# ross39/new_bloom_filter_repo

Hardware: AMD Instinct MI355X
Metric: Mpixels/s Bloom insert+query, 1080p residuals (higher is better)
Workload: dtype u64

## Files before the change

### include/rbf.h

```cpp
#ifndef RBF_H
#define RBF_H

#include <stddef.h>
#include <stdint.h>

#ifdef __cplusplus
extern "C" {
#endif

#define RBF_OK        0
#define RBF_EINVAL  (-22)
#define RBF_ENOMEM  (-12)
#define RBF_EIO      (-5)
#define RBF_ERANGE  (-34)

#define RBF_ABI_VERSION 4

typedef struct rbf_ctx rbf_ctx;

typedef struct {
    uint32_t m;
    uint32_t floor_k;
    uint64_t threshold;
} rbf_filter_params;

typedef struct {
    uint64_t h1;
    uint64_t h2;
    uint64_t act;
} rbf_seeds;

#define RBF_STAT_WITNESS_BITS 0
#define RBF_STAT_FILTER_ONES  1
#define RBF_STAT_RESERVED0    2
#define RBF_STAT_RESERVED1    3
#define RBF_STATS_PER_FRAME   4

int rbf_version(void);
const char *rbf_last_error(void);
int rbf_device_count(int *count);

int rbf_ctx_create(int device, void *hip_stream, rbf_ctx **out);
int rbf_ctx_destroy(rbf_ctx *ctx);
int rbf_ctx_sync(rbf_ctx *ctx);

int rbf_malloc(rbf_ctx *ctx, size_t bytes, void **out_dev);
int rbf_free(rbf_ctx *ctx, void *ptr_dev);
int rbf_memset(rbf_ctx *ctx, void *dst_dev, int value, size_t bytes);
int rbf_memcpy_h2d(rbf_ctx *ctx, void *dst_dev, const void *src, size_t bytes);
int rbf_memcpy_d2h(rbf_ctx *ctx, void *dst, const void *src_dev, size_t bytes);
int rbf_memcpy_d2d(rbf_ctx *ctx, void *dst_dev, const void *src_dev, size_t bytes);

#define RBF_K_MASK    0
#define RBF_K_INSERT  1
#define RBF_K_QUERY   2
#define RBF_K_STITCH  3
#define RBF_K_EXPAND  4
#define RBF_K_GATHER  5
#define RBF_K_SCATTER 6
#define RBF_K_INDEX   7
#define RBF_K_REDUCE  8
#define RBF_K_SCAN    9
#define RBF_K_NOISE   10
#define RBF_K_PACK    11
#define RBF_K_HASHTAB 12
#define RBF_K_HOLD    13
#define RBF_K_COUNT   14
int rbf_timing_enable(rbf_ctx *ctx, int on);
int rbf_ctx_force_generic(rbf_ctx *ctx, int on);
#define RBF_OPT_SEPARATE_FINISH 2
#define RBF_OPT_INSERT_SLICES 4
int rbf_ctx_option(rbf_ctx *ctx, int option, int64_t value);
int rbf_timing_reset(rbf_ctx *ctx);
int rbf_timing_read(rbf_ctx *ctx, int kernel_id, double *total_ms, uint64_t *launches);

int rbf_optimal_params(uint64_t n, uint64_t ones, double *k, uint64_t *l);
int rbf_activation_threshold(double k_star, uint32_t *floor_k, uint64_t *threshold);

int rbf_plan_batch(uint64_t n, const uint64_t *ones, uint32_t nframes, int guard_l_ge_n,
                   rbf_filter_params *params, double *k);

int rbf_residual_mask_batch(rbf_ctx *ctx, const void *frames_dev, uint64_t frame_stride_bytes,
                            uint32_t nframes, uint32_t width, uint32_t height,
                            uint64_t row_pitch_bytes, uint32_t pixel_stride_bytes,
                            uint32_t sample_bytes, int32_t thr_floor, const int32_t *thr_floors,
                            void *masks_dev, uint64_t mask_stride_bytes, uint64_t *ones_dev);

int rbf_residual_mask_batch_ex(rbf_ctx *ctx, const void *frames_dev, uint64_t frame_stride_bytes,
                               uint32_t nframes, uint32_t width, uint32_t height,
                               uint64_t row_pitch_bytes, uint32_t pixel_stride_bytes,
                               uint32_t sample_bytes, int32_t thr_floor, const int32_t *thr_floors,
                               void *masks_dev, uint64_t mask_stride_bytes, uint64_t *ones_dev, uint32_t mask_channels);

int rbf_temporal_hold_runs(rbf_ctx *ctx, void *frames_dev, uint64_t frame_stride_bytes, uint32_t nframes,
                           uint32_t width, uint32_t height, uint32_t channels, uint32_t sample_bytes,
                           uint32_t max_error, const uint8_t *run_starts);

int rbf_temporal_lookahead_runs(rbf_ctx *ctx, void *frames_dev, uint64_t frame_stride_bytes, uint32_t nframes,
                                uint32_t width, uint32_t height, uint32_t channels, uint32_t sample_bytes,
                                uint32_t max_error, const uint8_t *run_starts);

int rbf_temporal_hold_runs_map(rbf_ctx *ctx, void *frames_dev, uint64_t frame_stride_bytes, uint32_t nframes,
                               uint32_t width, uint32_t height, uint32_t channels, uint32_t sample_bytes,
                               const void *bounds_dev, const uint8_t *run_starts);
int rbf_temporal_lookahead_runs_map(rbf_ctx *ctx, void *frames_dev, uint64_t frame_stride_bytes, uint32_t nframes,
                                    uint32_t width, uint32_t height, uint32_t channels, uint32_t sample_bytes,
                                    const void *bounds_dev, const uint8_t *run_starts);

int rbf_bgr_to_gray_batch(rbf_ctx *ctx, const void *frames_dev, uint64_t frame_stride_bytes, uint32_t nframes,
                          uint32_t width, uint32_t height, uint64_t row_pitch_bytes, uint32_t pixel_stride_bytes,
                          uint32_t sample_bytes, void *gray_dev);

int rbf_extract_luma_batch(rbf_ctx *ctx, const void *frames_dev, uint64_t frame_stride_bytes, uint32_t nframes,
                           uint32_t width, uint32_t height, uint64_t row_pitch_bytes, uint32_t pixel_stride_bytes,
                           uint32_t sample_bytes, void *luma_dev);

int rbf_noise_moments_batch(rbf_ctx *ctx, const void *frames_dev, uint64_t frame_stride_bytes,
                            uint32_t nframes, uint32_t width, uint32_t height,
                            uint64_t row_pitch_bytes, uint32_t pixel_stride_bytes,
                            uint32_t sample_bytes, int64_t *moments_dev, float *noise_dev);


int rbf_bloom_encode_batch(rbf_ctx *ctx, const void *masks_dev, uint64_t mask_stride_bytes,
                           uint64_t n, uint32_t nframes, const rbf_filter_params *params,
                           const rbf_seeds *seeds,
                           void *filters_dev, uint64_t filter_stride_bytes,
                           void *witnesses_dev, uint64_t witness_stride_bytes,
                           uint64_t *stats_dev);

int rbf_encode_gop(rbf_ctx *ctx, const void *frames_dev, uint64_t frame_stride_bytes,
                   uint32_t nframes, uint32_t width, uint32_t height,
                   uint64_t row_pitch_bytes, uint32_t pixel_stride_bytes,
                   uint32_t sample_bytes, int32_t thr_floor, const int32_t *thr_floors,
                   const rbf_seeds *seeds,
                   void *masks_dev, uint64_t mask_stride_bytes, uint64_t *ones_dev,
                   void *filters_dev, uint64_t filter_stride_bytes,
                   void *witnesses_dev, uint64_t witness_stride_bytes, uint64_t *stats_dev,
                   rbf_filter_params *params_out, double *k_out);

int rbf_encode_gop_begin(rbf_ctx *ctx, const void *frames_dev, uint64_t frame_stride_bytes,
                         uint32_t nframes, uint32_t width, uint32_t height,
                         uint64_t row_pitch_bytes, uint32_t pixel_stride_bytes,
                         uint32_t sample_bytes, int32_t thr_floor, const int32_t *thr_floors,
                         const rbf_seeds *seeds,
                         void *masks_dev, uint64_t mask_stride_bytes, uint64_t *ones_dev,
                         void *filters_dev, uint64_t filter_stride_bytes,
                         void *witnesses_dev, uint64_t witness_stride_bytes, uint64_t *stats_dev);
int rbf_encode_gop_poll(rbf_ctx *ctx, int *ready);

#define RBF_PAIR_SKIPPED 0xFFFFFFFFu
uint64_t rbf_filter_stride_min(uint64_t n);
int rbf_encode_runs_begin(rbf_ctx *ctx, const void *frames_dev, uint64_t frame_stride_bytes,
                          uint32_t nframes, uint32_t width, uint32_t height,
                          uint64_t row_pitch_bytes, uint32_t pixel_stride_bytes,
// ... 118 lines not shown
```

### new_bloom_filter_repo_amd/_native.py

```python
import ctypes
import os
import weakref

import numpy as np

_HERE = os.path.dirname(os.path.abspath(__file__))
LIB_PATH = os.environ.get("RBF_LIB_PATH") or os.path.join(_HERE, "librbf_hip.so")

RBF_OK = 0
RBF_EINVAL = -22
RBF_ENOMEM = -12
RBF_EIO = -5
RBF_ERANGE = -34

K_MASK, K_INSERT, K_QUERY, K_STITCH, K_EXPAND, K_GATHER, K_SCATTER, K_INDEX, K_REDUCE, K_SCAN, K_NOISE, K_PACK, K_HASHTAB, K_HOLD = range(14)
KERNEL_NAMES = ["mask", "insert", "query", "stitch", "expand", "gather", "scatter", "index", "reduce", "scan", "noise", "pack", "hashtab", "hold"]
STATS_PER_FRAME = 4
PAIR_SKIPPED = 0xFFFFFFFF
OPT_SEPARATE_FINISH, OPT_INSERT_SLICES = 2, 4


class FilterParams(ctypes.Structure):
    _fields_ = [("m", ctypes.c_uint32), ("floor_k", ctypes.c_uint32), ("threshold", ctypes.c_uint64)]


ERROR_ROW = np.dtype([("sse", "<u8"), ("differing", "<u8"), ("over_bound", "<u8"), ("max_abs", "<u4"), ("reserved", "<u4")])
SWEEP_ROW = np.dtype([("sse", "<u8"), ("updates", "<u8"), ("max_abs", "<u4"), ("reserved", "<u4")])
SWEEP_MAX_CANDIDATES = 8
PAN_ROW = np.dtype([("dx", "<i4"), ("dy", "<i4"), ("sad_zero", "<u8"), ("sad_best", "<u8"), ("moving_zero", "<u8"), ("moving_best", "<u8")])
PAN_MAX_RANGE = 32


class Seeds(ctypes.Structure):
    _fields_ = [("h1", ctypes.c_uint64), ("h2", ctypes.c_uint64), ("act", ctypes.c_uint64)]


class RbfError(RuntimeError):
    def __init__(self, code, msg):
        super().__init__("librbf_hip error %d: %s" % (code, msg))
        self.code = code


_vp, _u64, _u32, _i32, _int = ctypes.c_void_p, ctypes.c_uint64, ctypes.c_uint32, ctypes.c_int32, ctypes.c_int
_i32p = ctypes.POINTER(ctypes.c_int32)
_PROTOS = {
    "rbf_version": (_int, []),
    "rbf_last_error": (ctypes.c_char_p, []),
    "rbf_device_count": (_int, [ctypes.POINTER(_int)]),
    "rbf_ctx_create": (_int, [_int, _vp, ctypes.POINTER(_vp)]),
    "rbf_ctx_destroy": (_int, [_vp]),
    "rbf_ctx_sync": (_int, [_vp]),
    "rbf_malloc": (_int, [_vp, ctypes.c_size_t, ctypes.POINTER(_vp)]),
    "rbf_free": (_int, [_vp, _vp]),
    "rbf_memset": (_int, [_vp, _vp, _int, ctypes.c_size_t]),
    "rbf_memcpy_h2d": (_int, [_vp, _vp, _vp, ctypes.c_size_t]),
    "rbf_memcpy_d2h": (_int, [_vp, _vp, _vp, ctypes.c_size_t]),
    "rbf_memcpy_d2d": (_int, [_vp, _vp, _vp, ctypes.c_size_t]),
    "rbf_timing_enable": (_int, [_vp, _int]),
    "rbf_timing_reset": (_int, [_vp]),
    "rbf_ctx_force_generic": (_int, [_vp, _int]),
    "rbf_ctx_option": (_int, [_vp, _int, ctypes.c_int64]),
    "rbf_timing_read": (_int, [_vp, _int, ctypes.POINTER(ctypes.c_double), ctypes.POINTER(_u64)]),
    "rbf_optimal_params": (_int, [_u64, _u64, ctypes.POINTER(ctypes.c_double), ctypes.POINTER(_u64)]),
    "rbf_activation_threshold": (_int, [ctypes.c_double, ctypes.POINTER(_u32), ctypes.POINTER(_u64)]),
    "rbf_plan_batch": (_int, [_u64, ctypes.POINTER(_u64), _u32, _int, ctypes.POINTER(FilterParams), ctypes.POINTER(ctypes.c_double)]),
    "rbf_encode_gop": (_int, [_vp, _vp, _u64, _u32, _u32, _u32, _u64, _u32, _u32, _i32, _i32p, ctypes.POINTER(Seeds),
                              _vp, _u64, _vp, _vp, _u64, _vp, _u64, _vp, ctypes.POINTER(FilterParams), ctypes.POINTER(ctypes.c_double)]),
    "rbf_encode_gop_begin": (_int, [_vp, _vp, _u64, _u32, _u32, _u32, _u64, _u32, _u32, _i32, _i32p, ctypes.POINTER(Seeds),
                                    _vp, _u64, _vp, _vp, _u64, _vp, _u64, _vp]),
    "rbf_encode_gop_poll": (_int, [_vp, ctypes.POINTER(_int)]),
    "rbf_filter_stride_min": (_u64, [_u64]),
    "rbf_encode_runs_begin": (_int, [_vp, _vp, _u64, _u32, _u32, _u32, _u64, _u32, _u32, _i32, _i32p, _vp, ctypes.POINTER(Seeds),
                                     _vp, _u64, _vp, _vp, _u64, _vp, _u64, _vp]),
    "rbf_encode_runs_begin_ex": (_int, [_vp, _vp, _u64, _u32, _u32, _u32, _u64, _u32, _u32, _i32, _i32p, _vp, ctypes.POINTER(Seeds),
                                        _vp, _u64, _vp, _vp, _u64, _vp, _u64, _vp, _u32]),
    "rbf_encode_runs": (_int, [_vp, _vp, _u64, _u32, _u32, _u32, _u64, _u32, _u32, _i32, _i32p, _vp, ctypes.POINTER(Seeds),
                               _vp, _u64, _vp, _vp, _u64, _vp, _u64, _vp, ctypes.POINTER(FilterParams), ctypes.POINTER(ctypes.c_double)]),
    "rbf_encode_gop_finish": (_int, [_vp, ctypes.POINTER(FilterParams), ctypes.POINTER(ctypes.c_double)]),
    "rbf_residual_mask_batch": (_int, [_vp, _vp, _u64, _u32, _u32, _u32, _u64, _u32, _u32, _i32, _i32p, _vp, _u64, _vp]),
    "rbf_residual_mask_batch_ex": (_int, [_vp, _vp, _u64, _u32, _u32, _u32, _u64, _u32, _u32, _i32, _i32p, _vp, _u64, _vp, _u32]),
    "rbf_temporal_hold_runs": (_int, [_vp, _vp, _u64, _u32, _u32, _u32, _u32, _u32, _u32, _vp]),
    "rbf_temporal_lookahead_runs": (_int, [_vp, _vp, _u64, _u32, _u32, _u32, _u32, _u32, _u32, _vp]),
    "rbf_temporal_hold_runs_map": (_int, [_vp, _vp, _u64, _u32, _u32, _u32, _u32, _u32, _vp, _vp]),
    "rbf_temporal_lookahead_runs_map": (_int, [_vp, _vp, _u64, _u32, _u32, _u32, _u32, _u32, _vp, _vp]),
    "rbf_record_max_bytes": (_u64, [_u32, _u64]),
    "rbf_pack_records": (_int, [_vp, _u32, _u64, ctypes.POINTER(FilterParams), ctypes.POINTER(ctypes.c_double),
                                _vp, _u64, _vp, _u64, _vp, _u64, _vp, _vp, _u64]),
    "rbf_gather_values_batch": (_int, [_vp, _vp, _u64, _u32, _u32, _u32, _u64, _u32, _u32, _u32, _vp, _u64, _vp, _u64, _vp, _vp]),
    "rbf_bgr_to_gray_batch": (_int, [_vp, _vp, _u64, _u32, _u32, _u32, _u64, _u32, _u32, _vp]),
    "rbf_extract_luma_batch": (_int, [_vp, _vp, _u64, _u32, _u32, _u32, _u64, _u32, _u32, _vp]),
    "rbf_noise_moments_batch": (_int, [_vp, _vp, _u64, _u32, _u32, _u32, _u64, _u32, _u32, _vp, _vp]),
    "rbf_bloom_encode_batch": (_int, [_vp, _vp, _u64, _u64, _u32, ctypes.POINTER(FilterParams), ctypes.POINTER(Seeds),
                                      _vp, _u64, _vp, _u64, _vp]),
    "rbf_bloom_decode_batch": (_int, [_vp, _vp, _u64, _vp, _u64, _u64, _u32, ctypes.POINTER(FilterParams),
                                      ctypes.POINTER(Seeds), _vp, _u64]),
    "rbf_filter_insert_indices": (_int, [_vp, _vp, ctypes.POINTER(FilterParams), ctypes.POINTER(Seeds), _vp, _u64]),
    "rbf_filter_query_indices": (_int, [_vp, _vp, ctypes.POINTER(FilterParams), ctypes.POINTER(Seeds), _vp, _u64, _vp]),
    "rbf_filter_insert_keys": (_int, [_vp, _vp, ctypes.POINTER(FilterParams), ctypes.POINTER(Seeds), _u32, _vp, _vp, _u64]),
    "rbf_filter_query_keys": (_int, [_vp, _vp, ctypes.POINTER(FilterParams), ctypes.POINTER(Seeds), _u32, _vp, _vp, _u64, _vp]),
    "rbf_gather_values": (_int, [_vp, _vp, _u32, _u32, _u64, _u32, _u32, _u32, _vp, _vp, _vp]),
    "rbf_scatter_values": (_int, [_vp, _vp, _u32, _u32, _u64, _u32, _u32, _u32, _vp, _vp]),
# ... 218 lines not shown
```

### new_bloom_filter_repo_amd/csrc/rbf_api.hip

```cpp
#include "rbf_host.h"
#include "rbf_kernels.h"
#include "rbf_kernels_noise.h"
#include "rbf_kernels_mask.h"
#include "rbf_kernels_hold.h"
#include "rbf_kernels_lookahead.h"
#include "rbf_kernels_barrett.h"
#include "rbf_kernels_insert_f64.h"
#include "rbf_kernels_reduce.h"
#include "rbf_kernels_query_f64.h"
#include "rbf_kernels_query_f64_tiled.h"
#include "rbf_kernels_witness.h"
#include "rbf_kernels_pack.h"
#include "rbf_kernels_digest.h"
#include "rbf_kernels_cut.h"
#include "rbf_kernels_error.h"
#include "rbf_kernels_sweep.h"
#include "rbf_kernels_pan.h"
#include "rbf_kernels_view.h"
#include "rbf_rice_host.h"
#include "rbf_kernels_keyquant.h"

#include <cmath>
#include <cstring>

// ... 341 lines not shown
            if (b.params[f].m) first += ones_host[f];
        }
        if (int r = launch_insert_positions(ctx, b, itab, sd, hashed_positions)) return r;
    }
    for (uint32_t f0 = 0; f0 < nframes;) {
        SliceTable grp{};
        uint32_t per_tile = 0, coded = 0, f = f0;
        for (; f < nframes && coded < pl.insert_group; ++f) {
            grp.n[f] = pl.slices.n[f];
            per_tile += grp.n[f];
            coded += grp.n[f] ? 1u : 0u;
        }
        f0 = f;
        if (!per_tile) continue;
        const dim3 grid(per_tile * pl.insert_tiles), block(IL_THREADS);
        LaunchTimer t(ctx, RBF_K_INSERT);
        if (two_phase)
            hipLaunchKernelGGL(k_insert_records, grid, block, pl.insert_lds_bytes, ctx->stream, (const uint2 *)ctx->ins_records.p,
                               (const uint32_t *)ctx->ins_counters.p, rtab, ctx->partials.p, part_stride, pl.insert_tile_words, grp, per_tile, pl.S);
        else if (use_tab)
            hipLaunchKernelGGL(tkern, grid, block, pl.insert_lds_bytes, ctx->stream, (const uint8_t *)b.masks, b.mask_stride, b.n, itab, hash_tab, sd,
                               ctx->partials.p, part_stride, pl.insert_tile_words, grp, per_tile, pl.S);
        else
            hipLaunchKernelGGL(ikern, grid, block, pl.insert_lds_bytes, ctx->stream, (const uint8_t *)b.masks, b.mask_stride, b.n, tab, sd,
                               ctx->partials.p, part_stride, pl.insert_tile_words, grp, per_tile, pl.S);
    }
    LaunchTimer t(ctx, RBF_K_REDUCE);
    const uint64_t words = b.filter_stride / 4;
    const uint32_t vec_ok = (words % 4 == 0 && ((uintptr_t)b.filters % 16) == 0) ? 1u : 0u;
    const uint32_t bx = std::max(1u, (uint32_t)((words + WG_THREADS * 4 - 1) / (WG_THREADS * 4)));
    hipLaunchKernelGGL(stream_once ? k_filter_reduce<true> : k_filter_reduce<false>, dim3(bx, nframes), dim3(WG_THREADS), 0, ctx->stream,
                       (const uint32_t *)ctx->partials.p, part_stride, pl.S, pl.slices, tab, (uint32_t *)b.filters, words, b.stats, vec_ok, image,
                       (uint64_t)pl.image_stride_words);
    return RBF_OK;
}

static int insert_generic(rbf_ctx *ctx, const Plan &pl, const BloomBatch &b, const FrameTable &tab, uint32_t *image)
{
    HIP_TRY(hipMemsetAsync(b.filters, 0, (size_t)b.nframes * b.filter_stride, ctx->stream));
    const uint64_t words = b.filter_stride / 4;
    const uint64_t bx = std::min<uint64_t>(((b.n + 31) / 32 + WG_THREADS - 1) / WG_THREADS, 65535);
    {
        LaunchTimer t(ctx, RBF_K_INSERT);
        hipLaunchKernelGGL(k_insert, dim3((uint32_t)bx, b.nframes), dim3(WG_THREADS), 0, ctx->stream, (const uint32_t *)b.masks, b.mask_stride / 4,
                           b.n, tab, to_dev(*b.seeds), (uint32_t *)b.filters, words);
    }
    LaunchTimer t(ctx, RBF_K_REDUCE);
    SliceTable ones;
    memset(ones.n, 1, sizeof ones.n);
    const uint32_t bx2 = std::max(1u, (uint32_t)((words + WG_THREADS * 4 - 1) / (WG_THREADS * 4)));
    hipLaunchKernelGGL(k_filter_reduce<false>, dim3(bx2, b.nframes), dim3(WG_THREADS), 0, ctx->stream, (const uint32_t *)b.filters, words, 1u, ones,
                       tab, (uint32_t *)b.filters, words, b.stats, 0u, image, (uint64_t)pl.image_stride_words);
    return RBF_OK;
}

static int encode_chunk_pass(rbf_ctx *ctx, const BloomBatch &b, bool outputs_zeroed, const uint64_t *ones_host, bool quiet_passthrough, bool compact)
{
    const uint32_t nframes = b.nframes;
    uint64_t nrecords = 0;
    uint32_t coded = 0;
    for (uint32_t f = 0; f < nframes; ++f) {
        if (!b.params[f].m) continue;
        ++coded;
        if (ones_host) nrecords += ones_host[f];
    }
    Plan pl = make_plan(ctx->knobs, ctx->cus, b.params, nframes, b.n, ones_host && nrecords < (1ull << 32));
    if (pl.insert_two_phase &&
        (ctx->ins_records.reserve((size_t)(nrecords ? nrecords : 1) * 8) || ctx->ins_counters.reserve((size_t)MAX_BATCH * 4))) {
        (void)hipGetLastError();
        pl = make_plan(ctx->knobs, ctx->cus, b.params, nframes, b.n, false);
    }
    FrameTable tab;
    if (int r = fill_table(b.params, nframes, &tab)) return r;
    const bool stream_once = (uint64_t)coded * b.n >= STREAM_MIN_PIXEL_FRAMES;
    if (int r = reserve_query_outputs(ctx, pl, nframes)) return r;
    if (int r = ctx->seg_off.reserve((size_t)nframes * pl.nseg * 8)) return r;
    const bool want_image = pl.reads_probe_image();
    if (want_image) if (int r = ctx->qimage.reserve((size_t)nframes * pl.image_stride_words * 4)) return r;
    uint32_t *image = want_image ? ctx->qimage.p : nullptr;
    if (!outputs_zeroed)
        HIP_TRY(hipMemsetAsync(b.stats, 0, (size_t)nframes * RBF_STATS_PER_FRAME * 8, ctx->stream));
    if (int r = pl.fast_insert ? insert_fast(ctx, pl, b, tab, ones_host, stream_once, image) : insert_generic(ctx, pl, b, tab, image)) return r;
    if (int r = launch_query(ctx, pl, b, tab, QueryFlags{want_image, pl.insert_tab, quiet_passthrough})) return r;
    if (compact) {
        uint32_t bx;
        if (int r = launch_chunk_offsets(ctx, pl, nframes, &bx, b.witnesses, b.witness_stride)) return r;
        LaunchTimer t(ctx, RBF_K_STITCH);
        hipLaunchKernelGGL(stream_once ? k_compact_witness<true> : k_compact_witness<false>, dim3(bx, nframes), dim3(WG_THREADS), 0, ctx->stream,
                           ctx->pass_words.p, ctx->seg_cnt.p, pl.nseg, pl.words_per_seg, (const uint64_t *)b.masks, b.mask_stride / 8, b.n,
                           (uint32_t *)b.witnesses, b.witness_stride / 4, b.stats, ctx->chunk_off.p);
    }
    HIP_TRY(hipGetLastError());
    return RBF_OK;
}

static int encode_chunk(rbf_ctx *ctx, const BloomBatch &b, bool outputs_zeroed, const uint64_t *ones_host)
{
    rbf_filter_params small[MAX_BATCH], big[MAX_BATCH];
    if (ctx->knobs.fp64_kernels() && !ctx->knobs.no_hash_table && split_by_family(b.params, b.nframes, small, big)) {
        const Plan ps = make_plan(ctx->knobs, ctx->cus, small, b.nframes, b.n, false);
        const Plan pb = make_plan(ctx->knobs, ctx->cus, big, b.nframes, b.n, ones_host != nullptr);
        if (pb.reads_probe_image() && pb.insert_tab && ps.nseg == pb.nseg && ps.words_per_seg == pb.words_per_seg) {
            if (int r = encode_chunk_pass(ctx, b.with(small), outputs_zeroed, nullptr, false, false)) return r;
            return encode_chunk_pass(ctx, b.with(big), true, ones_host, true, true);
        }
    }
    return encode_chunk_pass(ctx, b, outputs_zeroed, ones_host, false, true);
}

static int encode_batch_impl(rbf_ctx *ctx, const BloomBatch &b, bool outputs_zeroed, const uint64_t *ones_host = nullptr)
{
    if (int r = set_device(ctx)) return r;
    if (!b.masks || !b.params || !b.seeds || !b.filters || !b.witnesses || !b.stats) return fail(RBF_EINVAL, "null pointer");
    if (int r = check_frame_geometry(b.n, b.nframes, b.mask_stride)) return r;
    if (int r = check_filter_strides(b.params, b.nframes, b.filter_stride)) return r;
    if (int r = check_witness_stride(b.n, b.witness_stride)) return r;
    if (int r = check_base8(b.masks, "masks_dev")) return r;
    if (int r = check_base8(b.filters, "filters_dev")) return r;
    if (int r = check_base8(b.witnesses, "witnesses_dev")) return r;
    if (int r = check_base8(b.stats, "stats_dev")) return r;
    for (uint32_t f0 = 0; f0 < b.nframes; f0 += MAX_BATCH) {
        const uint32_t cnt = std::min(b.nframes - f0, (uint32_t)MAX_BATCH);
        if (int r = encode_chunk(ctx, b.rows(f0, cnt), outputs_zeroed, ones_host ? ones_host + f0 : nullptr)) return r;
    }
    return RBF_OK;
}

static int decode_chunk(rbf_ctx *ctx, const BloomBatch &b)
{
    const uint32_t nframes = b.nframes;
    const Plan pl = make_plan(ctx->knobs, ctx->cus, b.params, nframes, b.n);
    FrameTable tab;
    if (int r = fill_table(b.params, nframes, &tab)) return r;
    if (int r = reserve_query_outputs(ctx, pl, nframes)) return r;
    bool split = false;
    rbf_filter_params small[MAX_BATCH], big[MAX_BATCH];
    if (ctx->knobs.fp64_kernels() && split_by_family(b.params, nframes, small, big)) {
        const Plan ps = make_plan(ctx->knobs, ctx->cus, small, nframes, b.n), pb = make_plan(ctx->knobs, ctx->cus, big, nframes, b.n);
        if (pb.reads_probe_image() && ps.nseg == pl.nseg && pb.nseg == pl.nseg && ps.words_per_seg == pl.words_per_seg &&
            pb.words_per_seg == pl.words_per_seg) {
            FrameTable ts, tb;
            if (int r = fill_table(small, nframes, &ts)) return r;
            if (int r = fill_table(big, nframes, &tb)) return r;
            if (int r = launch_query(ctx, ps, b, ts, QueryFlags{})) return r;
            if (int r = launch_query(ctx, pb, b, tb, QueryFlags{false, false,  true})) return r;
            split = true;
        }
    }
    if (!split) if (int r = launch_query(ctx, pl, b, tab, QueryFlags{})) return r;
    uint32_t bx;
    if (int r = launch_chunk_offsets(ctx, pl, nframes, &bx)) return r;
    LaunchTimer t(ctx, RBF_K_EXPAND);
    hipLaunchKernelGGL(k_expand_mask, dim3(bx, nframes), dim3(WG_THREADS), 0, ctx->stream, ctx->pass_words.p, ctx->seg_cnt.p, pl.nseg,
                       pl.words_per_seg, (const uint32_t *)b.witnesses, b.witness_stride / 4, (uint64_t *)b.masks, b.mask_stride / 8, b.n,
                       ctx->chunk_off.p);
    HIP_TRY(hipGetLastError());
    return RBF_OK;
}

static LayoutRules frame_pass_rules(uint32_t samples)
{
    LayoutRules r;
    r.samples = samples; r.min_frames = 1; r.max_frames = 65535;
    return r;
}

template <class KernelOf>
// ... 116 lines not shown
    HIP_TRY(hipStreamSynchronize(ctx->stream));
    return RBF_OK;
}

int rbf_malloc(rbf_ctx *ctx, size_t bytes, void **out_dev)
{
    if (int r = set_device(ctx)) return r;
    if (!out_dev) return fail(RBF_EINVAL, "out_dev is null");
    *out_dev = nullptr;
    if (bytes == 0) bytes = 8;
    hipError_t e = hipMalloc(out_dev, bytes);
    if (e != hipSuccess) return fail(e == hipErrorOutOfMemory ? RBF_ENOMEM : RBF_EIO, "hipMalloc(%zu): %s", bytes, hipGetErrorString(e));
    return RBF_OK;
}

int rbf_free(rbf_ctx *ctx, void *ptr_dev)
{
    if (int r = set_device(ctx)) return r;
    if (!ptr_dev) return RBF_OK;
    HIP_TRY(hipStreamSynchronize(ctx->stream));
    HIP_TRY(hipFree(ptr_dev));
    return RBF_OK;
}

int rbf_memset(rbf_ctx *ctx, void *dst_dev, int value, size_t bytes)
{
    if (int r = set_device(ctx)) return r;
    if (bytes == 0) return RBF_OK;
    if (!dst_dev) return fail(RBF_EINVAL, "dst_dev is null");
    HIP_TRY(hipMemsetAsync(dst_dev, value, bytes, ctx->stream));
    return RBF_OK;
}

int rbf_memcpy_h2d(rbf_ctx *ctx, void *dst_dev, const void *src, size_t bytes)
{
    if (int r = set_device(ctx)) return r;
    if (bytes == 0) return RBF_OK;
    if (!dst_dev || !src) return fail(RBF_EINVAL, "null pointer");
    HIP_TRY(hipMemcpyAsync(dst_dev, src, bytes, hipMemcpyHostToDevice, ctx->stream));
    HIP_TRY(hipStreamSynchronize(ctx->stream));
    return RBF_OK;
}

int rbf_memcpy_d2h(rbf_ctx *ctx, void *dst, const void *src_dev, size_t bytes)
{
    if (int r = set_device(ctx)) return r;
    if (bytes == 0) return RBF_OK;
    if (!dst || !src_dev) return fail(RBF_EINVAL, "null pointer");
    HIP_TRY(hipMemcpyAsync(dst, src_dev, bytes, hipMemcpyDeviceToHost, ctx->stream));
    HIP_TRY(hipStreamSynchronize(ctx->stream));
    return RBF_OK;
}

int rbf_memcpy_d2d(rbf_ctx *ctx, void *dst_dev, const void *src_dev, size_t bytes)
{
    if (int r = set_device(ctx)) return r;
    if (bytes == 0) return RBF_OK;
    if (!dst_dev || !src_dev) return fail(RBF_EINVAL, "null pointer");
    HIP_TRY(hipMemcpyAsync(dst_dev, src_dev, bytes, hipMemcpyDeviceToDevice, ctx->stream));
    return RBF_OK;
}

int rbf_timing_enable(rbf_ctx *ctx, int on)
{
    if (int r = set_device(ctx)) return r;
    if (!on) { if (int r = drain_timing(ctx)) return r; }
    ctx->timing = on == 1 ? 0xFFFFFFFFu : (uint32_t)on;
    return RBF_OK;
}

int rbf_ctx_force_generic(rbf_ctx *ctx, int on)
{
    if (!ctx) return fail(RBF_EINVAL, "null context");
    ctx->knobs.set_flags(on);
    return RBF_OK;
}

int rbf_ctx_option(rbf_ctx *ctx, int option, int64_t value)
{
    if (!ctx) return fail(RBF_EINVAL, "null context");
    switch (option) {
    case RBF_OPT_SEPARATE_FINISH: ctx->knobs.no_fused_finish = value != 0; return RBF_OK;
    case RBF_OPT_INSERT_SLICES: ctx->knobs.insert_slices = value < 0 ? 0u : (uint32_t)value; return RBF_OK;
    default: return fail(RBF_EINVAL, "unknown option %d", option);
    }
}

int rbf_timing_reset(rbf_ctx *ctx)
{
    if (int r = set_device(ctx)) return r;
    if (int r = drain_timing(ctx)) return r;
    for (int k = 0; k < RBF_K_COUNT; ++k) { ctx->total_ms[k] = 0; ctx->launches[k] = 0; }
    return RBF_OK;
}

int rbf_timing_read(rbf_ctx *ctx, int kernel_id, double *total_ms, uint64_t *launches)
{
    if (int r = set_device(ctx)) return r;
    if (kernel_id < 0 || kernel_id >= RBF_K_COUNT) return fail(RBF_EINVAL, "kernel id %d", kernel_id);
    if (int r = drain_timing(ctx)) return r;
    if (total_ms) *total_ms = ctx->total_ms[kernel_id];
    if (launches) *launches = ctx->launches[kernel_id];
    return RBF_OK;
}

int rbf_optimal_params(uint64_t n, uint64_t ones, double *k_out, uint64_t *l_out)
{
    if (!k_out || !l_out) return fail(RBF_EINVAL, "null output");
    *k_out = 0.0; *l_out = 0;
    if (n == 0 || ones > n) return fail(RBF_EINVAL, "need 0 <= ones <= n, n > 0");
    const double p = (double)ones / (double)n;
    if (p <= 0.0001) return RBF_OK;
    if (p >= 0.32453) return RBF_OK;
    const double q = 1 - p;
    const double L = std::log(2.0);
    const double k = std::log2(q * std::pow(L, 2.0) / p);
    if (std::isnan(k) || k <= 0) return RBF_OK;
    const double gamma = 1 / L;
    const double lf = p * (double)n * k * gamma;
    const uint64_t l = (uint64_t)lf;
    *k_out = k > 0.1 ? k : 0.1;
    *l_out = l > 1 ? l : 1;
    return RBF_OK;
}

int rbf_activation_threshold(double k_star, uint32_t *floor_k, uint64_t *threshold)
{
    if (!floor_k || !threshold) return fail(RBF_EINVAL, "null output");
    if (!(k_star >= 0.0) || k_star > 64.0) return fail(RBF_ERANGE, "k* = %g outside [0, 64]", k_star);
    const double fl = std::floor(k_star);
    *floor_k = (uint32_t)fl;
    const double pa = k_star - fl;
    if (!(pa > 0.0)) { *threshold = 0; return RBF_OK; }
    int ex;
    const double fr = std::frexp(pa, &ex);
    const uint64_t A = (uint64_t)std::ldexp(fr, 53);
    const int s = ex - 53 - 2;
    const uint64_t N = (A == (1ull << 52)) ? 4 * A - 1 : 4 * A - 2;
    const int sh = -s;
    if (sh >= 128) { *threshold = 1; return RBF_OK; }
    const unsigned __int128 X = (unsigned __int128)N * (unsigned __int128)0xFFFFFFFFFFFFFFFFull;
    *threshold = (uint64_t)(X >> sh) + 1;
    return RBF_OK;
}

int rbf_plan_batch(uint64_t n, const uint64_t *ones, uint32_t nframes, int guard_l_ge_n,
                   rbf_filter_params *params, double *k_out)
{
    if (!ones || !params) return fail(RBF_EINVAL, "null pointer");
    for (uint32_t f = 0; f < nframes; ++f) {
        double k = 0.0; uint64_t l = 0;
        if (int r = rbf_optimal_params(n, ones[f], &k, &l)) return r;
        const bool skip = (l == 0) || (guard_l_ge_n && l >= n) || l > 0xFFFFFFFFull;
        params[f].m = 0; params[f].floor_k = 0; params[f].threshold = 0;
        if (!skip) {
            params[f].m = (uint32_t)l;
            if (int r = rbf_activation_threshold(k, &params[f].floor_k, &params[f].threshold)) return r;
        }
        if (k_out) k_out[f] = skip ? 0.0 : k;
    }
    return RBF_OK;
}

int rbf_residual_mask_batch(rbf_ctx *ctx, const void *frames_dev, uint64_t frame_stride_bytes,
                            uint32_t nframes, uint32_t width, uint32_t height,
                            uint64_t row_pitch_bytes, uint32_t pixel_stride_bytes,
// ... 1070 lines not shown
```

### new_bloom_filter_repo_amd/csrc/rbf_kernels_witness.h

```cpp
#pragma once
#include "rbf_kernels.h"

namespace rbf {

constexpr int CO_THREADS = 1024;
__global__ __launch_bounds__(CO_THREADS) void k_chunk_offsets(const uint32_t *__restrict__ seg_cnt, uint64_t nseg, uint32_t chunk_segs, uint32_t nchunks,
                                                              uint32_t *__restrict__ off, uint32_t *__restrict__ witnesses , uint64_t witness_stride_words32)
{
    __shared__ uint32_t wtot[CO_THREADS / WAVE];
    __shared__ uint32_t carry_s;
    const uint32_t f = blockIdx.x;
    const uint32_t lane = threadIdx.x & 63u, wave = threadIdx.x >> 6;
    const uint32_t *cnt = seg_cnt + (uint64_t)f * nseg;
    uint32_t *out = off + (uint64_t)f * nchunks;
    uint32_t *wit = witnesses ? witnesses + (uint64_t)f * witness_stride_words32 : nullptr;
    auto zero_word_at = [&](uint32_t bit) {
        const uint64_t d = (bit >> 5) & ~1u;
        if (d < witness_stride_words32) wit[d] = 0;
        if (d + 1 < witness_stride_words32) wit[d + 1] = 0;
    };
    const uint32_t per = (chunk_segs & 3u) == 0 ? 4u : (chunk_segs & 1u) == 0 ? 2u : 1u;
    if (threadIdx.x == 0) carry_s = 0;
    __syncthreads();
    for (uint64_t base = 0; base < nseg; base += (uint64_t)CO_THREADS * per) {
// ... 61 lines not shown
        off += __popc(p4);
    }
    return out;
}
__device__ __forceinline__ uint32_t pdep32_lut(const uint8_t *lut, uint32_t w, uint32_t p)
{
    uint32_t out = 0, off = 0;
#pragma unroll
    for (int j = 0; j < 8; ++j) {
        const uint32_t p4 = __builtin_amdgcn_ubfe(p, 4u * j, 4u), w4 = __builtin_amdgcn_ubfe(w, off, 4u);
        out |= (uint32_t)lut[(p4 << 4) | w4] << (4u * j);
        off += __popc(p4);
    }
    return out;
}

template <bool STREAM>
__global__ __launch_bounds__(WG_THREADS) void k_compact_witness(
    const uint64_t *__restrict__ pass_words, const uint32_t *__restrict__ seg_cnt, uint64_t nseg, uint32_t words_per_seg,
    const uint64_t *__restrict__ masks, uint64_t mask_stride_words64, uint64_t n,
    uint32_t *__restrict__ witnesses, uint64_t witness_stride_words32, uint64_t *__restrict__ stats,
    const uint32_t *__restrict__ chunk_off )
{
    __shared__ uint32_t buf[WG_THREADS * 2 + 2];
    __shared__ uint32_t wsum[WG_WAVES];
    __shared__ __attribute__((aligned(4))) uint8_t lut[256];
    const uint32_t f = blockIdx.y;
    const uint32_t lane = threadIdx.x & 63u, wave = __builtin_amdgcn_readfirstlane(threadIdx.x >> 6);
    const uint32_t nwords = (uint32_t)((n + 63) >> 6);
    const uint32_t total = (uint32_t)nseg * words_per_seg;
    const uint64_t *pwf = pass_words + (uint64_t)f * total;
    const uint32_t start32 = chunk_off[(uint64_t)f * gridDim.x + blockIdx.x];
    uint32_t *wit = witnesses + (uint64_t)f * witness_stride_words32;
    const uint32_t wbeg = blockIdx.x * WG_THREADS;
    const uint32_t w = wbeg + threadIdx.x;
    const bool have = w < total && w < nwords;
    const uint64_t *mkp = masks + (uint64_t)f * mask_stride_words64 + w;
    const uint64_t pw_raw = have ? (STREAM ? __builtin_nontemporal_load(pwf + w) : pwf[w]) : 0ull;
    const uint64_t mk_raw = have ? (STREAM ? __builtin_nontemporal_load(mkp) : *mkp) : 0ull;
    lut_to_lds(lut, LUT_PEXT4);
    buf[threadIdx.x] = 0;
    buf[threadIdx.x + WG_THREADS] = 0;
    if (threadIdx.x < 2) buf[threadIdx.x + 2 * WG_THREADS] = 0;
    const uint64_t pw = flip_bytes64(pw_raw);
    const uint32_t pw_lo = (uint32_t)pw, pw_hi = (uint32_t)(pw >> 32);
    const uint32_t c_lo = __popc(pw_lo), c = c_lo + __popc(pw_hi);
    const uint32_t incl = wave_inclusive_scan(c);
    if (lane == WAVE - 1) wsum[wave] = incl;
    __syncthreads();
    uint32_t before = 0, chunk_total = 0;
#pragma unroll
    for (int k = 0; k < WG_WAVES; ++k) {
        if ((uint32_t)k < wave) before += wsum[k];
        chunk_total += wsum[k];
    }
    const uint32_t obase = start32 & ~31u;
    const uint32_t o = start32 + before + incl - c;
    const uint64_t mk = flip_bytes64(mk_raw);
    const uint32_t o_lo = pext32_lut(lut, (uint32_t)mk, pw_lo), o_hi = pext32_lut(lut, (uint32_t)(mk >> 32), pw_hi);
    const uint64_t out = (uint64_t)o_lo | ((uint64_t)o_hi << c_lo);
    if (out) {
        const uint32_t rel = o - obase;
        const uint32_t sh = rel & 31u, word = rel >> 5;
        const uint32_t lo = (uint32_t)out, hi = (uint32_t)(out >> 32);
        const uint32_t d0 = lo << sh;
        const uint32_t d1 = sh ? ((lo >> (32u - sh)) | (hi << sh)) : hi;
        const uint32_t d2 = sh ? (hi >> (32u - sh)) : 0u;
        if (d0) atomicOr(&buf[word], d0);
        if (d1) atomicOr(&buf[word + 1], d1);
        if (d2) atomicOr(&buf[word + 2], d2);
    }
    __syncthreads();
    const uint32_t oend = start32 + chunk_total;
    const uint32_t ndw = ((oend - obase) + 31u) >> 5;
    for (uint32_t i = threadIdx.x; i < ndw; i += WG_THREADS) {
        const uint32_t v = buf[i];
        const bool shared = (i == 0 && (start32 & 31u)) || (i + 1 == ndw && (oend & 31u));
        if (shared) { if (v) atomicOr(&wit[(obase >> 5) + i], flip_bytes32(v)); }
        else wit[(obase >> 5) + i] = flip_bytes32(v);
    }
    if (threadIdx.x == 0 && wbeg + WG_THREADS >= total) stats[(uint64_t)f * 4 + 0] = oend;
}

__global__ __launch_bounds__(WG_THREADS) void k_expand_mask(
    const uint64_t *__restrict__ pass_words, const uint32_t *__restrict__ seg_cnt, uint64_t nseg, uint32_t words_per_seg,
    const uint32_t *__restrict__ witnesses, uint64_t witness_stride_words32,
    uint64_t *__restrict__ masks, uint64_t mask_stride_words64, uint64_t n, const uint32_t *__restrict__ chunk_off )
{
    __shared__ uint32_t wsum[WG_WAVES];
    __shared__ __attribute__((aligned(4))) uint8_t lut[256];
    const uint32_t f = blockIdx.y;
    const uint32_t lane = threadIdx.x & 63u, wave = __builtin_amdgcn_readfirstlane(threadIdx.x >> 6);
    const uint32_t nwords = (uint32_t)((n + 63) >> 6);
    const uint32_t total = (uint32_t)nseg * words_per_seg;
    const uint32_t start32 = chunk_off[(uint64_t)f * gridDim.x + blockIdx.x];
    const uint32_t *wit = witnesses + (uint64_t)f * witness_stride_words32;
    const uint32_t wbeg = blockIdx.x * WG_THREADS;
    const uint32_t w = wbeg + threadIdx.x;
    const bool have = w < total && w < nwords;
    const uint64_t pw_raw = have ? pass_words[(uint64_t)f * total + w] : 0ull;
    lut_to_lds(lut, LUT_PDEP4);
    const uint64_t p = flip_bytes64(pw_raw);
    const uint32_t p_lo = (uint32_t)p, p_hi = (uint32_t)(p >> 32);
    const uint32_t c_lo = __popc(p_lo), c = c_lo + __popc(p_hi);
    const uint32_t incl = wave_inclusive_scan(c);
    if (lane == WAVE - 1) wsum[wave] = incl;
    __syncthreads();
    uint32_t o = start32 + incl - c;
#pragma unroll
    for (int k = 0; k < WG_WAVES; ++k)
        if ((uint32_t)k < wave) o += wsum[k];
    if (w >= nwords) return;
    uint64_t out = 0;
    if (c) {
        const uint32_t d0 = o >> 5, dl = (o + c - 1u) >> 5, r = o & 31u;
        const uint64_t x0 = d0 < witness_stride_words32 ? flip_bytes32(wit[d0]) : 0u;
        const uint64_t x1 = (d0 + 1 <= dl && d0 + 1 < witness_stride_words32) ? flip_bytes32(wit[d0 + 1]) : 0u;
        const uint64_t x2 = (d0 + 2 <= dl && d0 + 2 < witness_stride_words32) ? flip_bytes32(wit[d0 + 2]) : 0u;
        uint64_t win = (x0 | (x1 << 32)) >> r;
        win |= r ? x2 << (64u - r) : 0ull;
        out = (uint64_t)pdep32_lut(lut, (uint32_t)win, p_lo) | ((uint64_t)pdep32_lut(lut, (uint32_t)(win >> c_lo), p_hi) << 32);
    }
    masks[(uint64_t)f * mask_stride_words64 + w] = flip_bytes64(out);
}

}
```

### new_bloom_filter_repo_amd/csrc/rbf_plan.h

```cpp
#pragma once
#include "../../include/rbf.h"
#include "rbf_geometry.h"

#include <algorithm>
#include <cstring>

using namespace rbf;

static int fail(int code, const char *fmt, ...);

struct Knobs {
    bool force_generic = false;
    bool single_buffer = false;
    bool force_generic_mask_bits = false;
    bool barrett_only = false;
    bool hash_rebuild = false;
    bool no_hash_table = false;
    bool no_two_phase = false;
    bool hash_positions = false;
    bool no_table_rewrite = false;
    bool no_fused_finish = false;
    uint32_t mask_chunks = 0;
    uint32_t tile_words = 0;
    uint32_t insert_slices = 0;
    void set_flags(int on)
    {
        force_generic = on & 1;
        single_buffer = on & 2;
        force_generic_mask_bits = on & 4;
        barrett_only = on & 8;
        hash_rebuild = on & 16;
        no_hash_table = on & 32;
        no_two_phase = on & 128;
        mask_chunks = (uint32_t)(on >> 8) & 0x1F;
        hash_positions = on & (1 << 14);
        no_table_rewrite = on & (1 << 15);
        tile_words = ((uint32_t)on >> 16) << 6;
    }
    bool fp64_kernels() const { return !force_generic && !barrett_only && !single_buffer; }
};

static inline FrameDev frame_dev(const rbf_filter_params &p)
{
    return FrameDev{p.m, p.floor_k, p.threshold, p.m >= 2 ? (uint64_t)((((unsigned __int128)1) << 64) / p.m) : 0};
}

static int fill_table(const rbf_filter_params *params, uint32_t count, FrameTable *tab)
{
    memset(tab, 0, sizeof *tab);
    for (uint32_t f = 0; f < count; ++f) {
        if (params[f].floor_k > 64) return fail(RBF_ERANGE, "frame %u: floor_k %u > 64", f, params[f].floor_k);
        tab->f[f] = frame_dev(params[f]);
    }
    return RBF_OK;
}

static FrameTable query_table(const FrameTable &tab, uint32_t nframes, U64Classes *cls, uint32_t *nactive, uint64_t (&empty)[2])
{
    FrameTable q;
    memset(&q, 0, sizeof q);
    if (cls) memset(cls, 0, sizeof *cls);
    empty[0] = empty[1] = 0;
    uint64_t sorted[MAX_BATCH];
    uint32_t coded = 0;
    for (uint32_t f = 0; f < nframes; ++f) {
        if (tab.f[f].m) sorted[coded++] = tab.f[f].T;
        else empty[f >> 6] |= 1ull << (f & 63);
    }
    std::sort(sorted, sorted + coded);
    uint32_t j = 0;
    for (int k = 0; k < (cls ? U64_CLASSES : 1); ++k)
        for (uint32_t f = 0; f < nframes; ++f) {
            if (!tab.f[f].m) continue;
            const uint32_t fk = tab.f[f].floor_k;
            if (cls && (fk >= 1u && fk <= 5u ? (int)fk - 1 : 5) != k) continue;
            const double ninv = -1.0 / (double)tab.f[f].m;
            const uint32_t below = (uint32_t)(std::lower_bound(sorted, sorted + coded, tab.f[f].T) - sorted);
            q.f[j].m = tab.f[f].m;
            memcpy(&q.f[j].M, &ninv, 8);
            q.f[j].floor_k = (fk & 0xFFu) | (below << 8) | (f << 16);
            q.f[j].T = sorted[j];
            if (cls) ++cls->n[k];
            ++j;
        }
    *nactive = coded;
    return q;
}

constexpr size_t LDS_LIMIT = 160 * 1024;
constexpr size_t HASH_TABLE_CACHE_BYTES = (size_t)96 << 20;
constexpr uint32_t MAX_INSERT_TILES = 7, MAX_QUERY_TILES = 3;
constexpr uint64_t STREAM_MIN_PIXEL_FRAMES = 64ull * 1920 * 1080;

enum class QueryKind {
    Generic,
    LdsWhole,
    LdsTiled,
    LdsTiledF64,
};

struct Plan {
    bool fast_insert;
    QueryKind query;
    bool double_buffer, small_m;
    bool insert_tab;
    bool insert_two_phase;
    bool f64_mod;
    uint32_t fwords_max, S , per_tile , insert_group ;
    SliceTable slices;
    uint32_t insert_tile_words, insert_tiles, query_tile_words;
    size_t insert_lds_bytes, query_lds_bytes;
    uint64_t nseg; uint32_t words_per_seg;
    uint32_t image_stride_words;
    bool reads_probe_image() const { return (query == QueryKind::LdsWhole || query == QueryKind::LdsTiledF64) && f64_mod; }
};

static inline uint32_t round_up4(uint32_t words) { return (words + 3u) & ~3u; }
static inline bool in_f64_range(uint32_t m) { return m >= F64MOD_M_MIN && m <= F64MOD_M_MAX; }
static inline size_t hash_table_bytes(uint64_t n) { return ((size_t)n + QL_SEG_PIXELS) * 32; }

static uint32_t tile_words_for(uint32_t fwords, uint32_t cap, uint32_t knob, bool even)
{
    uint32_t tw = round_up4(fwords);
    if (tw > cap) {
        const uint32_t nt = (fwords + cap - 1) / cap;
        tw = even ? round_up4((fwords + nt - 1) / nt) : cap;
    }
    if (knob && knob < tw) tw = knob & ~3u;
    return tw < 4 ? 4 : tw;
}

struct BatchSizes {
    uint32_t mmax = 0, active = 0;
    bool small_m = true;
    bool all_f64 = true;
};

static BatchSizes classify(const rbf_filter_params *params, uint32_t nframes)
{
    BatchSizes b;
    for (uint32_t f = 0; f < nframes; ++f) {
        const uint32_t m = params[f].m;
        if (m > b.mmax) b.mmax = m;
        if (m) ++b.active;
        if (m == 1 || m > (1u << 30)) b.small_m = false;
        if (m && !in_f64_range(m)) b.all_f64 = false;
    }
    return b;
}

static void plan_insert_tiles(Plan &p, const Knobs &k, const BatchSizes &b, bool have_ones)
{
    const size_t queue_bytes = (size_t)IL_WAVES * (IT_WAVE_LDS_BYTES > IL_QUEUE * 4 ? IT_WAVE_LDS_BYTES : IL_QUEUE * 4);
    p.insert_tile_words = tile_words_for(p.fwords_max, (uint32_t)((LDS_LIMIT - queue_bytes) / 4) & ~3u, k.tile_words, false);
    p.insert_lds_bytes = (size_t)p.insert_tile_words * 4 + queue_bytes;
    p.insert_tiles = std::max(1u, (p.fwords_max + p.insert_tile_words - 1) / p.insert_tile_words);
    p.fast_insert = !k.force_generic && b.mmax > 0 && !(k.tile_words == 0 && p.insert_tiles > MAX_INSERT_TILES);
    p.insert_tab = p.fast_insert && b.all_f64 && !k.no_hash_table && !k.barrett_only;
    p.insert_two_phase = p.insert_tab && !k.no_two_phase && have_ones && p.insert_tiles > 1;
    if (p.insert_two_phase) {
        p.insert_tile_words = tile_words_for(p.fwords_max, (uint32_t)(LDS_LIMIT / 4) & ~3u, k.tile_words, true);
        p.insert_tiles = (p.fwords_max + p.insert_tile_words - 1) / p.insert_tile_words;
        p.insert_lds_bytes = (size_t)p.insert_tile_words * 4;
    }
}

static void plan_query(Plan &p, const Knobs &k, const BatchSizes &b, uint32_t nframes, uint64_t n)
{
    const size_t fbytes = (size_t)round_up4(p.fwords_max) * 4;
    const bool lds = !k.force_generic && b.mmax > 0;
    const bool u64_offsets_fit = (uint64_t)nframes * ((n + QL_SEG_PIXELS - 1) / QL_SEG_PIXELS) * (QL_SEG_PIXELS / 8) < (1ull << 32);
    p.f64_mod = b.all_f64 && !k.barrett_only && !k.single_buffer && u64_offsets_fit &&
                2 * (fbytes + 16) + u64_geo_bytes(nframes) <= LDS_LIMIT;
    const size_t qbytes = fbytes + (p.f64_mod ? 16 : 0);
    p.double_buffer = 2 * qbytes <= LDS_LIMIT && !k.single_buffer;
    p.query = QueryKind::Generic;
    if (lds && qbytes <= LDS_LIMIT && !k.tile_words) {
        p.query = QueryKind::LdsWhole;
        p.query_lds_bytes = (p.double_buffer ? 2 : 1) * qbytes;
    } else if (lds) {
        p.query = QueryKind::LdsTiled;
        p.query_tile_words = (uint32_t)(LDS_LIMIT / 4);
        if (k.tile_words && k.tile_words < p.query_tile_words) p.query_tile_words = k.tile_words & ~3u;
        if (p.query_tile_words < 4) p.query_tile_words = 4;
        p.query_lds_bytes = (size_t)std::min(p.query_tile_words, round_up4(p.fwords_max)) * 4;
        if (k.tile_words == 0 && (p.fwords_max + p.query_tile_words - 1) / p.query_tile_words > MAX_QUERY_TILES) p.query = QueryKind::Generic;
    }
    if (lds && b.all_f64 && !k.barrett_only && !k.single_buffer && !p.reads_probe_image()) {
        const uint32_t cap = (uint32_t)((LDS_LIMIT - S64_GEO_BYTES) / 4 - 4) & ~3u;
        p.query = QueryKind::LdsTiledF64;
        p.query_tile_words = tile_words_for(p.fwords_max, cap, k.tile_words, true);
        p.query_lds_bytes = (size_t)(p.query_tile_words + 4) * 4;
        p.f64_mod = true;
    }
    if (p.query != QueryKind::LdsWhole && p.query != QueryKind::LdsTiledF64) p.f64_mod = false;
    const uint32_t segpx = p.query == QueryKind::LdsWhole || p.query == QueryKind::LdsTiledF64 ? (uint32_t)QL_SEG_PIXELS
                         : p.query == QueryKind::LdsTiled ? (uint32_t)TQ_SEG_PIXELS : (uint32_t)SEG_PIXELS;
    p.nseg = (n + segpx - 1) / segpx;
    p.words_per_seg = segpx / 64;
}

static void plan_slices(Plan &p, const Knobs &k, uint32_t cus, uint32_t active, const rbf_filter_params *params, uint32_t nframes)
{
    constexpr uint32_t INSERT_SLICES = 8;
    const uint32_t units = std::max(1u, cus / p.insert_tiles);
    uint32_t group = std::max(1u, units / INSERT_SLICES);
    if (group > active) group = active ? active : 1;
    uint32_t base = std::min(std::max(1u, units / group), 32u);
    if (p.insert_tiles == 1 && !p.insert_two_phase && active) {
        group = active;
        base = 1;
        while (base * 2 * active <= units && base < 32) base *= 2;
        if (k.insert_slices) base = std::min(k.insert_slices, 32u);
    }
    p.insert_group = group;
    p.S = base;
    p.per_tile = 0;
    for (uint32_t f = 0; f < nframes; ++f) {
        const uint32_t sf = params[f].m ? base : 0u;
        p.slices.n[f] = (uint8_t)sf;
        p.per_tile += sf;
    }
}

static Plan make_plan(const Knobs &k, uint32_t cus, const rbf_filter_params *params, uint32_t nframes, uint64_t n, bool have_ones = false)
{
    Plan p{};
    const BatchSizes b = classify(params, nframes);
    p.small_m = b.small_m;
    p.fwords_max = (uint32_t)(((uint64_t)b.mmax + 31) / 32);
    p.image_stride_words = round_up4(p.fwords_max);
    plan_insert_tiles(p, k, b, have_ones);
    plan_query(p, k, b, nframes, n);
    plan_slices(p, k, cus, b.active, params, nframes);
    return p;
}

static bool split_by_family(const rbf_filter_params *params, uint32_t nframes, rbf_filter_params *small, rbf_filter_params *big)
{
    uint32_t in_range = 0, out_of_range = 0;
    for (uint32_t f = 0; f < nframes; ++f) {
        small[f] = big[f] = params[f];
        if (!params[f].m) continue;
        ++(in_f64_range(params[f].m) ? in_range : out_of_range);
        (in_f64_range(params[f].m) ? small[f] : big[f]).m = 0;
    }
    return in_range && out_of_range;
}
```

Baseline: 556,700.

## Fuse witness compaction offsets into single span-based kernel

Measured after the change: 564,300 (median of 6 runs). +1.4%, better.

```diff
diff --git a/include/rbf.h b/include/rbf.h
--- a/include/rbf.h
+++ b/include/rbf.h
@@ -70,6 +70,8 @@
 int rbf_ctx_force_generic(rbf_ctx *ctx, int on);
 #define RBF_OPT_SEPARATE_FINISH 2
 #define RBF_OPT_INSERT_SLICES 4
+#define RBF_OPT_COMPACT_PAIR  6
+#define RBF_OPT_COMPACT_SPANS 7
 int rbf_ctx_option(rbf_ctx *ctx, int option, int64_t value);
 int rbf_timing_reset(rbf_ctx *ctx);
 int rbf_timing_read(rbf_ctx *ctx, int kernel_id, double *total_ms, uint64_t *launches);
diff --git a/new_bloom_filter_repo_amd/_native.py b/new_bloom_filter_repo_amd/_native.py
--- a/new_bloom_filter_repo_amd/_native.py
+++ b/new_bloom_filter_repo_amd/_native.py
@@ -17,6 +17,7 @@
 KERNEL_NAMES = ["mask", "insert", "query", "stitch", "expand", "gather", "scatter", "index", "reduce", "scan", "noise", "pack", "hashtab", "hold"]
 STATS_PER_FRAME = 4
 PAIR_SKIPPED = 0xFFFFFFFF
+OPT_COMPACT_PAIR, OPT_COMPACT_SPANS = 6, 7
 OPT_SEPARATE_FINISH, OPT_INSERT_SLICES = 2, 4
 
 
diff --git a/new_bloom_filter_repo_amd/csrc/rbf_api.hip b/new_bloom_filter_repo_amd/csrc/rbf_api.hip
--- a/new_bloom_filter_repo_amd/csrc/rbf_api.hip
+++ b/new_bloom_filter_repo_amd/csrc/rbf_api.hip
@@ -447,7 +447,12 @@
         HIP_TRY(hipMemsetAsync(b.stats, 0, (size_t)nframes * RBF_STATS_PER_FRAME * 8, ctx->stream));
     if (int r = pl.fast_insert ? insert_fast(ctx, pl, b, tab, ones_host, stream_once, image) : insert_generic(ctx, pl, b, tab, image)) return r;
     if (int r = launch_query(ctx, pl, b, tab, QueryFlags{want_image, pl.insert_tab, quiet_passthrough})) return r;
-    if (compact) {
+    if (compact && !ctx->knobs.compact_pair) {
+        LaunchTimer t(ctx, RBF_K_STITCH);
+        hipLaunchKernelGGL(stream_once ? k_compact_witness_fused<true> : k_compact_witness_fused<false>, dim3(pl.compact_spans, nframes),
+                           dim3(WG_THREADS), 0, ctx->stream, ctx->pass_words.p, ctx->seg_cnt.p, pl.nseg, pl.words_per_seg, (const uint64_t *)b.masks,
+                           b.mask_stride / 8, b.n, (uint32_t *)b.witnesses, b.witness_stride / 4, b.stats, pl.compact_chunks);
+    } else if (compact) {
         uint32_t bx;
         if (int r = launch_chunk_offsets(ctx, pl, nframes, &bx, b.witnesses, b.witness_stride)) return r;
         LaunchTimer t(ctx, RBF_K_STITCH);
@@ -730,6 +735,8 @@
     switch (option) {
     case RBF_OPT_SEPARATE_FINISH: ctx->knobs.no_fused_finish = value != 0; return RBF_OK;
     case RBF_OPT_INSERT_SLICES: ctx->knobs.insert_slices = value < 0 ? 0u : (uint32_t)value; return RBF_OK;
+    case RBF_OPT_COMPACT_PAIR: ctx->knobs.compact_pair = value != 0; return RBF_OK;
+    case RBF_OPT_COMPACT_SPANS: ctx->knobs.compact_spans = value < 0 ? 0u : (uint32_t)std::min<int64_t>(value, 65535); return RBF_OK;
     default: return fail(RBF_EINVAL, "unknown option %d", option);
     }
 }
diff --git a/new_bloom_filter_repo_amd/csrc/rbf_kernels_witness.h b/new_bloom_filter_repo_amd/csrc/rbf_kernels_witness.h
--- a/new_bloom_filter_repo_amd/csrc/rbf_kernels_witness.h
+++ b/new_bloom_filter_repo_amd/csrc/rbf_kernels_witness.h
@@ -167,6 +167,133 @@
     if (threadIdx.x == 0 && wbeg + WG_THREADS >= total) stats[(uint64_t)f * 4 + 0] = oend;
 }
 
+__host__ __device__ constexpr uint32_t compact_span_begin(uint32_t g, uint32_t G, uint32_t nchunks) { return (uint32_t)((uint64_t)g * nchunks / G); }
+
+template <bool STREAM>
+__global__ __launch_bounds__(WG_THREADS) void k_compact_witness_fused(
+    const uint64_t *__restrict__ pass_words, const uint32_t *__restrict__ seg_cnt, uint64_t nseg, uint32_t words_per_seg,
+    const uint64_t *__restrict__ masks, uint64_t mask_stride_words64, uint64_t n,
+    uint32_t *__restrict__ witnesses, uint64_t witness_stride_words32, uint64_t *__restrict__ stats, uint32_t nchunks)
+{
+    __shared__ uint32_t buf[WG_THREADS * 2 + 2];
+    __shared__ uint32_t wsum[WG_WAVES];
+    __shared__ __attribute__((aligned(4))) uint8_t lut[256];
+    const uint32_t f = blockIdx.y, g = blockIdx.x, G = gridDim.x;
+    const uint32_t lane = threadIdx.x & 63u, wave = __builtin_amdgcn_readfirstlane(threadIdx.x >> 6);
+    const uint32_t nwords = (uint32_t)((n + 63) >> 6);
+    const uint32_t total = (uint32_t)nseg * words_per_seg;
+    const uint32_t have_end = total < nwords ? total : nwords;
+    const uint64_t *pwf = pass_words + (uint64_t)f * total;
+    const uint64_t *mkf = masks + (uint64_t)f * mask_stride_words64;
+    uint32_t *wit = witnesses + (uint64_t)f * witness_stride_words32;
+    const uint32_t c0 = compact_span_begin(g, G, nchunks), c1 = compact_span_begin(g + 1, G, nchunks);
+    auto load_pass = [&](uint32_t w) { return w < have_end ? (STREAM ? __builtin_nontemporal_load(pwf + w) : pwf[w]) : 0ull; };
+    auto load_mask = [&](uint32_t w) { return w < have_end ? (STREAM ? __builtin_nontemporal_load(mkf + w) : mkf[w]) : 0ull; };
+    uint64_t pw_raw = load_pass(c0 * WG_THREADS + threadIdx.x), mk_raw = load_mask(c0 * WG_THREADS + threadIdx.x);
+    uint64_t wp_raw = c0 ? load_pass(c0 * WG_THREADS - 1u - threadIdx.x) : 0ull, wx_raw = c0 ? load_mask(c0 * WG_THREADS - 1u - threadIdx.x) : 0ull;
+    lut_to_lds(lut, LUT_PEXT4);
+    buf[threadIdx.x] = 0;
+    buf[threadIdx.x + WG_THREADS] = 0;
+    if (threadIdx.x < 2) buf[threadIdx.x + 2 * WG_THREADS] = 0;
+    uint32_t b0;
+    {
+        const uint32_t *cnt = seg_cnt + (uint64_t)f * nseg;
+        const uint64_t segs = (uint64_t)c0 * (WG_THREADS / words_per_seg);
+        const uint32_t nbefore = (uint32_t)(segs < nseg ? segs : nseg);
+        uint32_t sum = 0;
+        for (uint32_t i = threadIdx.x; i < nbefore; i += WG_THREADS) sum += cnt[i];
+        const uint32_t incl = wave_inclusive_scan(sum);
+        if (lane == WAVE - 1) wsum[wave] = incl;
+        __syncthreads();
+        b0 = 0;
+#pragma unroll
+        for (int k = 0; k < WG_WAVES; ++k) b0 += wsum[k];
+        __syncthreads();
+    }
+    const uint32_t need = b0 & 31u;
+    for (uint32_t got = 0, wend = c0 * WG_THREADS; got < need && wend > 0;) {
+        const uint64_t p = flip_bytes64(wp_raw), x = flip_bytes64(wx_raw);
+        const uint32_t p_lo = (uint32_t)p, p_hi = (uint32_t)(p >> 32);
+        const uint32_t c_lo = __popc(p_lo), c = c_lo + __popc(p_hi);
+        const uint32_t incl = wave_inclusive_scan(c);
+        if (lane == WAVE - 1) wsum[wave] = incl;
+        __syncthreads();
+        uint32_t after = got + incl - c, batch = 0;
+#pragma unroll
+        for (int k = 0; k < WG_WAVES; ++k) {
+            if ((uint32_t)k < wave) after += wsum[k];
+            batch += wsum[k];
+        }
+        if (c && after < need) {
+            const uint64_t out = (uint64_t)pext32_lut(lut, (uint32_t)x, p_lo) | ((uint64_t)pext32_lut(lut, (uint32_t)(x >> 32), p_hi) << c_lo);
+            const int at = (int)need - (int)after - (int)c;
+            const uint32_t v = (uint32_t)(at >= 0 ? out << at : out >> -at) & ((1u << need) - 1u);
+            if (v) atomicOr(&buf[0], v);
+        }
+        got += batch;
+        wend -= WG_THREADS;
+        if (got < need && wend > 0) {
+            wp_raw = load_pass(wend - 1u - threadIdx.x);
+            wx_raw = load_mask(wend - 1u - threadIdx.x);
+        }
+        __syncthreads();
+    }
+    uint32_t cur = b0;
+    for (uint32_t ch = c0; ch < c1; ++ch) {
+        const bool more = ch + 1 < c1;
+        const uint32_t wn = (ch + 1) * WG_THREADS + threadIdx.x;
+        const uint64_t pw_next = more ? load_pass(wn) : 0ull, mk_next = more ? load_mask(wn) : 0ull;
+        const uint64_t pw = flip_bytes64(pw_raw);
+        const uint32_t pw_lo = (uint32_t)pw, pw_hi = (uint32_t)(pw >> 32);
+        const uint32_t c_lo = __popc(pw_lo), c = c_lo + __popc(pw_hi);
+        const uint32_t incl = wave_inclusive_scan(c);
+        if (lane == WAVE - 1) wsum[wave] = incl;
+        __syncthreads();
+        uint32_t before = 0, chunk_total = 0;
+#pragma unroll
+        for (int k = 0; k < WG_WAVES; ++k) {
+            if ((uint32_t)k < wave) before += wsum[k];
+            chunk_total += wsum[k];
+        }
+        const uint32_t obase = cur & ~31u;
+        const uint32_t o = cur + before + incl - c;
+        const uint64_t mk = flip_bytes64(mk_raw);
+        const uint32_t o_lo = pext32_lut(lut, (uint32_t)mk, pw_lo), o_hi = pext32_lut(lut, (uint32_t)(mk >> 32), pw_hi);
+        const uint64_t out = (uint64_t)o_lo | ((uint64_t)o_hi << c_lo);
+        if (out) {
+            const uint32_t rel = o - obase;
+            const uint32_t sh = rel & 31u, word = rel >> 5;
+            const uint32_t lo = (uint32_t)out, hi = (uint32_t)(out >> 32);
+            const uint32_t d0 = lo << sh;
+            const uint32_t d1 = sh ? ((lo >> (32u - sh)) | (hi << sh)) : hi;
+            const uint32_t d2 = sh ? (hi >> (32u - sh)) : 0u;
+            if (d0) atomicOr(&buf[word], d0);
+            if (d1) atomicOr(&buf[word + 1], d1);
+            if (d2) atomicOr(&buf[word + 2], d2);
+        }
+        __syncthreads();
+        const uint32_t oend = cur + chunk_total;
+        const uint32_t nfull = (oend >> 5) - (obase >> 5);
+        for (uint32_t i = threadIdx.x; i < nfull; i += WG_THREADS) {
+            wit[(obase >> 5) + i] = flip_bytes32(buf[i]);
+            buf[i] = 0;
+        }
+        if (threadIdx.x == 0 && nfull) {
+            buf[0] = buf[nfull];
+            buf[nfull] = 0;
+        }
+        cur = oend;
+        pw_raw = pw_next;
+        mk_raw = mk_next;
+    }
+    if (g + 1 != G) return;
+    if (threadIdx.x == 0) stats[(uint64_t)f * 4 + 0] = cur;
+    if ((cur & 63u) && threadIdx.x < 2) {
+        const uint32_t d = (cur >> 5) + threadIdx.x;
+        if (d <= ((cur - 1u) >> 5 | 1u) && d < witness_stride_words32) wit[d] = threadIdx.x == 0 ? flip_bytes32(buf[0]) : 0u;
+    }
+}
+
 __global__ __launch_bounds__(WG_THREADS) void k_expand_mask(
     const uint64_t *__restrict__ pass_words, const uint32_t *__restrict__ seg_cnt, uint64_t nseg, uint32_t words_per_seg,
     const uint32_t *__restrict__ witnesses, uint64_t witness_stride_words32,
diff --git a/new_bloom_filter_repo_amd/csrc/rbf_plan.h b/new_bloom_filter_repo_amd/csrc/rbf_plan.h
--- a/new_bloom_filter_repo_amd/csrc/rbf_plan.h
+++ b/new_bloom_filter_repo_amd/csrc/rbf_plan.h
@@ -23,6 +23,8 @@
     uint32_t mask_chunks = 0;
     uint32_t tile_words = 0;
     uint32_t insert_slices = 0;
+    bool compact_pair = false;
+    uint32_t compact_spans = 0;
     void set_flags(int on)
     {
         force_generic = on & 1;
@@ -112,6 +114,7 @@
     size_t insert_lds_bytes, query_lds_bytes;
     uint64_t nseg; uint32_t words_per_seg;
     uint32_t image_stride_words;
+    uint32_t compact_chunks, compact_spans;
     bool reads_probe_image() const { return (query == QueryKind::LdsWhole || query == QueryKind::LdsTiledF64) && f64_mod; }
 };
 
@@ -223,6 +226,14 @@
     }
 }
 
+constexpr uint32_t COMPACT_WG_PER_CU = 2;
+static void plan_compaction(Plan &p, const Knobs &k, uint32_t cus, uint32_t active)
+{
+    p.compact_chunks = (uint32_t)std::max<uint64_t>(1, (p.nseg * p.words_per_seg + WG_THREADS - 1) / WG_THREADS);
+    const uint32_t want = k.compact_spans ? k.compact_spans : COMPACT_WG_PER_CU * cus / std::max(1u, active);
+    p.compact_spans = std::min(std::max(1u, want), p.compact_chunks);
+}
+
 static Plan make_plan(const Knobs &k, uint32_t cus, const rbf_filter_params *params, uint32_t nframes, uint64_t n, bool have_ones = false)
 {
     Plan p{};
@@ -233,6 +244,7 @@
     plan_insert_tiles(p, k, b, have_ones);
     plan_query(p, k, b, nframes, n);
     plan_slices(p, k, cus, b.active, params, nframes);
+    plan_compaction(p, k, cus, b.active);
     return p;
 }
 
```
